# nv-dvl/nerfmatch

Hardware: AMD Instinct MI355X
Metric: rays*samples/sec (higher is better)
Workload: dtype fp16x3 (fp16 MFMA on hi/lo-split fp32 operands, three products per fp32 product, fp32 accumulate; fp32 everywhere else)

## Files before the change

nerfmatch_amd/csrc/nerf_fwd_bf16.hip:

```cpp
#include "nerf_split_chain.h"

namespace {
using namespace nmbf;
using nmsample::HALF_PI_F32, nmsample::SCAN_TILE, nmsample::frustum, nmsample::ray_consts, nmsample::lift_var, nmsample::ipe_fast, nmsample::view_row_value;
using nmsample::alpha_of, nmsample::trans_factor, nmsample::sigmoid, nmsample::scan_before_barrier, nmsample::scan_after_barrier, nmsample::scan_carry;
using nmsample::first_max;
static_assert(TILE == SCAN_TILE, "the compositing scan of nerf_sample.h spans two wavefronts");

template <int PART>
__device__ __forceinline__ void tap_prefetch(Ctx& cx) {
  if constexpr (PART == 0) __builtin_amdgcn_s_barrier();
  const char* src = reinterpret_cast<const char*>(cx.tapw);
#pragma unroll
  for (int q = (PART == 0 ? 0 : 4); q < (PART == 0 ? 4 : 7); ++q) {
    const char* sp = src + q * 4096;
    const float* dp = q < 4 ? cx.tap_ring + q * 1024 : cx.tap_ipe + (q - 4) * 1024;
    const unsigned lds = (unsigned)__builtin_amdgcn_readfirstlane((int)(unsigned)(size_t)(const __attribute__((address_space(3))) float*)dp);
    unsigned m0_saved;
    asm volatile("s_mov_b32 %0, m0\n\ts_mov_b32 m0, %1\n\tglobal_load_lds_dwordx4 %2, off\n\tglobal_load_lds_dwordx4 %2, off offset:1024\n\t"
                 "global_load_lds_dwordx4 %2, off offset:2048\n\tglobal_load_lds_dwordx4 %2, off offset:3072\n\ts_mov_b32 m0, %0"
                 : "=&s"(m0_saved) : "s"(lds), "v"(sp) : "memory");
  }
}

// ... 57 lines not shown
#pragma unroll
    for (int i = 0; i < 8; ++i) s2[8 * b + i] = o[i];
  }
  float s3[16];
#pragma unroll
  for (int b = 0; b < 2; ++b) {
    float o[8], x[8], y[8];
#pragma unroll
    for (int i = 0; i < 8; ++i) { x[i] = s2[8 * b + i]; y[i] = s2[16 + 8 * b + i]; }
    dpp_pairs8(o, x, y, false);
#pragma unroll
    for (int i = 0; i < 8; ++i) s3[8 * b + i] = o[i];
  }
  float lo8[8], hi8[8];
#pragma unroll
  for (int i = 0; i < 8; ++i) { lo8[i] = s3[i]; hi8[i] = s3[8 + i]; }
  quad_add8<2>(lo8); quad_add8<2>(hi8);
  float s4[8];
#pragma unroll
  for (int i = 0; i < 8; ++i) s4[i] = (lane & 2) ? hi8[i] : lo8[i];
  float t8[8] = {s4[0], s4[1], s4[2], s4[3], s4[4], s4[5], s4[6], s4[7]};
  quad_add8<1>(t8);
  return (lane & 1) ? f32x4{t8[4], t8[5], t8[6], t8[7]} : f32x4{t8[0], t8[1], t8[2], t8[3]};
}
__device__ __forceinline__ f32x4 reduce_scatter_32rows(float (&v)[128], int lane) {
  float s1[64];
#pragma unroll
  for (int i = 0; i < 64; ++i) s1[i] = reduce_scatter_step16(v[i], v[64 + i]);
  return reduce_scatter_16pairs(s1, lane);
}

#define NM_MLP_DONE_WAIT() __builtin_amdgcn_s_waitcnt(0x0070)
#define NM_EPI_BARRIER() asm volatile("s_waitcnt lgkmcnt(0)\n\ts_barrier" ::: "memory")
template <int P, bool TAP7 = true>
__device__ __forceinline__ void nerf_fwd_body(const NerfArgs& a) {
  constexpr bool DENS = P == 2 && !TAP7;
  __shared__ __attribute__((aligned(16))) float sm[LDS_TOTAL];
  float* const sm_small = sm + LDS_SMALL;
  float* const ring = sm + LDS_RING;
  float* const sm_ipe = sm + LDS_IPE;
  float* const sm_sigma = sm + LDS_SCR;
  float* const sm_rgb = sm_sigma + TILE;
  float* const sm_t0 = sm_rgb + 3 * TILE;
  float* const sm_t1 = sm_t0 + TILE;
  float* const sm_mean = sm_t1 + TILE;
  float* const sm_dn = sm_mean + 3 * TILE;
  float* const sm_w = sm_dn + TILE;
  float* const sm_misc = sm_w + TILE;
  float* const sm_part = sm_misc + 32;
  float* const sm_feat = sm + LDS_FEAT;
  float* const sm_ex = sm + LDS_EX;
  int* const sm_lray = reinterpret_cast<int*>(sm + LDS_LEFT);
  float* const sm_lT = sm + LDS_LEFT + TILE;
  unsigned* const sm_rng = reinterpret_cast<unsigned*>(sm + LDS_RNG);

  const int tid = threadIdx.x, lane = tid & 63, wave = tid >> 6, s = lane & 31, hi = lane >> 5;
  const bool tail_ok = a.left && !(a.tail_viol && *a.tail_viol != 0);
  const int S = a.S, R = a.R;
  const int Sa = tail_ok ? a.Sa : S;
  const int left = tail_ok ? 1 : 0;
  const int ntiles = tail_ok ? a.ntiles : a.ntiles_full;
  const int SP = Sa < TILE ? Sa : TILE;
  const int nr = TILE / SP;
  const int nchunks = (Sa + TILE - 1) / TILE;
  const bool need_rgb = !(a.flags & NM_NERF_SKIP_RGB);
  const bool feat_max = (a.flags & NM_NERF_FEAT_MAX) != 0;
  const bool need_tap = (a.feat != nullptr) || (a.sfeat != nullptr);
  const int tap = (a.tap < 0 || a.tap > 7) ? 7 : a.tap;
  const int nslots = need_rgb ? NSLOT_FULL : NSLOT_NORGB;
// ... 48 lines not shown
    const float t0 = a.t[(size_t)rc * (S + 1) + sidx];
    const float t1 = a.t[(size_t)rc * (S + 1) + sidx + 1];
    float t_mean, t_var, r_var;
    frustum(t0, t1, radius, t_mean, t_var, r_var);
    float mean[3] = {d0 * t_mean + o0, d1 * t_mean + o1, d2 * t_mean + o2};
    float var[3];
    lift_var(t_var, r_var, dsq, nul, a.var_scale, var);
    if (hi == 0) {
      sm_t0[js] = t0; sm_t1[js] = t1;
      sm_mean[js] = mean[0]; sm_mean[TILE + js] = mean[1]; sm_mean[2 * TILE + js] = mean[2];
      sm_dn[js] = dnorm;
    }

    ring_open<P>(blob_slots, ring, wave, lane);

    {
      const float ipe_scale = sm_small[OFF_INSCALE];
      const float phl = hi ? HALF_PI_F32 : 0.f;
      park_ipe<P>(sm_ipe + wave * (XS * 2 * 64 * 4) + lane * 4, [&](int idx) {
        const int ax = idx % 3;
        const float sc = (float)(1 << (idx / 3));
        float v = ipe_fast(mean[ax] * sc + phl, var[ax], sc);
        if constexpr (P == 2) v *= ipe_scale;
        return v;
      });
    }

    TRACE(2);
    Ctx cx;
    cx.blob_slots = blob_slots; cx.ring = ring; cx.sm_small = sm_small;
    cx.tapw = reinterpret_cast<f32x4*>(a.ws) + ((size_t)blockIdx.x * 4 + wave) * 32 * 64 + lane;
    cx.nslots = nslots; cx.wave = wave; cx.lane = lane; cx.hi = hi; cx.tap = need_tap ? tap : -1; cx.g = 0; cx.sig_part = 0.f;
    cx.vmax = 0.f; cx.rng = sm_rng + tid; cx.sc = 1.f;
    const bool early = TAP7 && need_rgb && !lo_pass && tap == 7 && a.feat && !a.sfeat;
    cx.tap_pref = need_tap && !lo_pass && !early; cx.rgb = need_rgb;
    cx.tap_ring = ring + wave * SLOT_FLOATS; cx.tap_ipe = sm_ipe + wave * (XS * 2 * 64 * 4);
    if constexpr (is_split<P>()) {
      ring_open_wait<P>(cx);
    } else {
      ring_acquire<P>(blob_slots, 0, nslots, ring, wave, lane);
    }
    load_half<P>(cx.opA, ring, lane, 0);
    if constexpr (P == 1) load_half<1>(cx.opB, ring, lane, 1);
    const float* ipe_src = sm_ipe + wave * (XS * 2 * 64 * 4) + lane * 4;

    auto composite_weights = [&]() __attribute__((always_inline)) {
      const int tid2 = launder(threadIdx.x), lane2 = tid2 & 63, wave2 = tid2 >> 6;
      float alpha = 0.f, incl = 1.f;
      if (tid2 < TILE) {
        alpha = alpha_of(sm_sigma[tid2], (sm_t1[tid2] - sm_t0[tid2]) * sm_dn[tid2]);
        incl = scan_before_barrier(trans_factor(alpha), lane2, wave2, SP, sm_misc);
      }
      NM_EPI_BARRIER();
      if (tid2 < TILE) {
        const float excl = scan_after_barrier(incl, lane2, wave2, SP, sm_misc, carryT);
        sm_w[tid2] = alpha * excl;
        const int r2 = tid2 / SP, ray2 = bid * nr + r2;
        if (left && chunk == nchunks - 1 && ray2 < R && tid2 % SP == SP - 1) {
          sm_lray[nleft + r2] = ray2;
          sm_lT[nleft + r2] = excl * trans_factor(alpha);
        }
      }
      if (nchunks > 1) carryT = scan_carry(carryT, sm_misc);
    };
    auto composite_sums = [&]() __attribute__((always_inline)) {
      const int tid2 = launder(threadIdx.x);
      if (tid2 < TILE) {
        const float wgt = sm_w[tid2];
        const int r2 = tid2 / SP, ray2 = bid * nr + r2;
        if (ray2 < R) {
          const int s2 = chunk * TILE + tid2 % SP;
          a.weights[(size_t)ray2 * S + s2] = wgt;
          if (left && chunk == nchunks - 1) {
            for (int k = Sa + 1 + tid2 % SP; k < S; k += SP) a.weights[(size_t)ray2 * S + k] = 0.f;
          }
          if (a.raw && !NM_TRACE) {
            f32x4 rv = {sm_rgb[tid2], sm_rgb[TILE + tid2], sm_rgb[2 * TILE + tid2], sm_sigma[tid2]};
            *reinterpret_cast<f32x4*>(a.raw + ((size_t)ray2 * S + s2) * 4) = rv;
          }
        }
        float pq[8] = {wgt, wgt * sm_rgb[tid2], wgt * sm_rgb[TILE + tid2], wgt * sm_rgb[2 * TILE + tid2],
                       wgt * (0.5f * (sm_t0[tid2] + sm_t1[tid2])), wgt * sm_mean[tid2], wgt * sm_mean[TILE + tid2],
                       wgt * sm_mean[2 * TILE + tid2]};
        nm_half_sum_dpp8(pq);
        if ((tid2 & 31) == 16) {
          *reinterpret_cast<f32x4*>(sm_part + (tid2 >> 5) * 8) = f32x4{pq[0], pq[1], pq[2], pq[3]};
          *reinterpret_cast<f32x4*>(sm_part + (tid2 >> 5) * 8 + 4) = f32x4{pq[4], pq[5], pq[6], pq[7]};
        }
      }
    };
    auto pick_best = [&]() __attribute__((always_inline)) {
      const int tid2 = launder(threadIdx.x);
      if (tid2 < 8 * nr) {
        const int q = tid2 & 7, r2 = tid2 >> 3;
        const float* wv = sm_w + r2 * SP;
        int bi;
        const bool better = first_max(wv, SP, best_w, bi);
        if (q == 0) sm_misc[8 + r2] = better ? __int_as_float(r2 * SP + bi) : __int_as_float(-1);
        if (q >= 5 && better) red_acc = sm_mean[(q - 5) * TILE + r2 * SP + bi];
      }
    };
    auto tap7_early = [&](Ctx& c) __attribute__((always_inline)) {
      const int t2 = launder(threadIdx.x), jl = (t2 >> 6) * 32 + (t2 & 31), hl = (t2 >> 5) & 1;
      const float sigma_raw = (c.sig_part + nm_shfl_xor32(c.sig_part)) + sm_small[OFF_MISC];
      if (hl == 0) sm_sigma[jl] = sigma_raw;
      NM_EPI_BARRIER();
      composite_weights();
      NM_EPI_BARRIER();
      if (feat_max) {
        pick_best();
        NM_EPI_BARRIER();
      }
      const float desc = sm_small[OFF_DESCALE + 7];
      const float wj = sm_w[jl] * desc;
      const int best = feat_max ? __float_as_int(sm_misc[8 + jl / SP]) : -2;
      const float mult = feat_max ? (jl == best ? desc : 0.f) : wj;
      const float* bl = sm_small + OFF_BIAS + 7 * 256 + 4 * hl;
      const float s7 = sm_small[OFF_SCALE + 7];
      float s1[64];
#pragma unroll
      for (int cq = 0; cq < HS; ++cq) {
        const f32x4 b0 = *reinterpret_cast<const f32x4*>(bl + (cq >> 2) * 32 + 8 * (cq & 3));
        const f32x4 b1 = *reinterpret_cast<const f32x4*>(bl + (4 + (cq >> 2)) * 32 + 8 * (cq & 3));
#pragma unroll
        for (int e = 0; e < 4; ++e) {
          const float x = mult * __builtin_fmaxf(__builtin_fmaf(c.hv[4 * cq + e], s7, b0[e]), 0.f);
          const float y = mult * __builtin_fmaxf(__builtin_fmaf(c.hv[64 + 4 * cq + e], s7, b1[e]), 0.f);
          s1[4 * cq + e] = reduce_scatter_step16(x, y);
        }
      }
      const f32x4 sum4 = reduce_scatter_16pairs(s1, jl);
      const int r = jl & 31;
      float* prow = sm_feat + (jl >> 5) * 256 + 4 * hl;
      *reinterpret_cast<f32x4*>(prow + (r >> 2) * 32 + 16 * ((r >> 1) & 1) + 8 * (r & 1)) = sum4;
    };
    const Tap7InRegisters<decltype(tap7_early)> tap7{early, tap7_early};
    f32x16 acc[8];
    ipe_steps<P, true>(acc, cx, ipe_src);
    finish_layer<P>(acc, 0, cx);
    TRACE(3);
#pragma unroll 1
    for (int l = 1; l < 8; ++l) {
      layer_pass<P, DENS>(acc, l, cx, ipe_src, tap7);
      TRACE(3 + l);
    }
    float c_r = 0.f, c_g = 0.f, c_b = 0.f;
    if (!need_rgb) {
      if (cx.tap == 7) dump_tap(7, cx);
      NM_MLP_DONE_WAIT();
      if (cx.tap_pref) tap_prefetch<0>(cx);
      alpha_head(cx);
      if (cx.tap_pref) tap_prefetch<1>(cx);
    } else {
      const int hh = launder(lane) >> 5;
      const float* exr = sm_ex + launder(rl) * 48 + 8 * hh;
      f32x16 av[4];
      if constexpr (DENS) {
        views_hidden<P, true>(av, cx);
        dens_close(cx);
      } else views_hidden<P>(av, cx);
      fold_range<P>(cx, 7);
      bf16x8 exh[VS], exl[VS];
#pragma unroll
      for (int e = 0; e < VS; ++e) {
        float v8[8];
        if (!lo_pass) {
          const f32x4 e0 = *reinterpret_cast<const f32x4*>(exr + 16 * e), e1 = *reinterpret_cast<const f32x4*>(exr + 16 * e + 4);
          v8[0] = e0[0]; v8[1] = e0[1]; v8[2] = e0[2]; v8[3] = e0[3]; v8[4] = e1[0]; v8[5] = e1[1]; v8[6] = e1[2]; v8[7] = e1[3];
        } else {
          const float* rq = a.rays + (size_t)launder(rc) * 12 + 8;
          const float vd0 = rq[0], vd1 = rq[1], vd2 = rq[2];
#pragma unroll
          for (int i = 0; i < 8; ++i) {
            const int f = 16 * e + 8 * hh + i;
            const int ax = f % 3;
            float v = view_row_value(f, ax == 0 ? vd0 : ax == 1 ? vd1 : vd2, a.app_row);
// ... 68 lines not shown
      }
      __syncthreads();
      if (need_tap) {
        const int jl = launder(js), hl = launder(lane) >> 5;
        const f32x4* tw = reinterpret_cast<const f32x4*>(a.ws) + ((size_t)blockIdx.x * 4 + wave2) * 32 * 64 + lane2;
        if (jl < nent) {
          const int ray2 = sm_lray[jl];
          const float desc = sm_small[OFF_DESCALE + tap];
          const float wj = sm_w[jl] * desc;
#pragma unroll 4
          for (int ks = 0; ks < HS; ++ks) {
            const f32x4 ta = tw[(2 * ks) * 64], tb = tw[(2 * ks + 1) * 64];
            const int n0 = (ks >> 1) * 32 + 16 * (ks & 1) + 4 * hl;
            if (a.sfeat) {
              float* dsf = a.sfeat + ((size_t)ray2 * S + Sa) * 256 + n0;
              *reinterpret_cast<f32x4*>(dsf) = ta * desc;
              *reinterpret_cast<f32x4*>(dsf + 8) = tb * desc;
            }
            if (a.feat) {
              float* df = a.feat + (size_t)ray2 * 256 + n0;
#pragma unroll
              for (int e = 0; e < 4; ++e) {
                atomicAdd(df + e, wj * ta[e]);
                atomicAdd(df + 8 + e, wj * tb[e]);
              }
            }
          }
        }
      }
      __syncthreads();
      break;
    }

    if (!early) composite_weights();
    composite_sums();
    NM_EPI_BARRIER();

    if (tid2 < 8 * nr) {
      const int q = tid2 & 7, r2 = tid2 >> 3;
      if (!feat_max || q < 5) {
        float sum = 0.f;
        for (int hw = r2 * (SP / 32); hw < (r2 + 1) * (SP / 32); ++hw) sum += sm_part[hw * 8 + q];
        red_acc += sum;
      }
    }
    if (feat_max && !early) {
      pick_best();
      NM_EPI_BARRIER();
    }

    TRACE(14);
    if (need_tap && !early) {
      const int jl = launder(js), hl = launder(lane) >> 5;
      f32x4 tapv[2 * HS];
      {
        asm volatile("s_waitcnt vmcnt(0)" ::: "memory");
        f32x4 tail[4];
        {
          const f32x4* tw = reinterpret_cast<const f32x4*>(a.ws) + ((size_t)blockIdx.x * 4 + (launder(threadIdx.x) >> 6)) * 32 * 64 + (launder(threadIdx.x) & 63);
#pragma unroll
          for (int i = 0; i < 4; ++i) tail[i] = tw[(28 + i) * 64];
        }
        const float* lr = ring + (launder(threadIdx.x) >> 6) * SLOT_FLOATS + (launder(threadIdx.x) & 63) * 4;
        const float* li = sm_ipe + (launder(threadIdx.x) >> 6) * (XS * 2 * 64 * 4) + (launder(threadIdx.x) & 63) * 4;
#pragma unroll
        for (int c = 0; c < 2 * HS; ++c)
          tapv[c] = c < 16 ? *reinterpret_cast<const f32x4*>(lr + c * 256) : c < 28 ? *reinterpret_cast<const f32x4*>(li + (c - 16) * 256) : tail[c - 28];
      }
      const float desc = sm_small[OFF_DESCALE + tap];
      const float wj = sm_w[jl] * desc;
      const int rsel = jl / SP;
      const int best = feat_max ? __float_as_int(sm_misc[8 + rsel]) : -2;
      float* prow = sm_feat + (jl >> 5) * 256 + 4 * hl;
      if (a.sfeat && ray < R) {
#pragma unroll
        for (int ks = 0; ks < HS; ++ks) {
          const f32x4 ta = tapv[2 * ks], tb = tapv[2 * ks + 1];
          float* dsf = a.sfeat + ((size_t)ray * S + sidx) * 256 + (ks >> 1) * 32 + 16 * (ks & 1) + 4 * hl;
          *reinterpret_cast<f32x4*>(dsf) = ta * desc;
          *reinterpret_cast<f32x4*>(dsf + 8) = tb * desc;
        }
      }
      if (a.feat) {
        float wv[128];
        const float mult = feat_max ? (jl == best ? desc : 0.f) : wj;
#pragma unroll
        for (int c = 0; c < 2 * HS; ++c)
#pragma unroll
          for (int e = 0; e < 4; ++e) wv[4 * c + e] = mult * tapv[c][e];
        const f32x4 sum4 = reduce_scatter_32rows(wv, jl);
        const int r = jl & 31;
        *reinterpret_cast<f32x4*>(prow + (r >> 2) * 32 + 16 * ((r >> 1) & 1) + 8 * (r & 1)) = sum4;
      }
    }
    TRACE(15);
    __syncthreads();
    TRACE(16);
    if (a.feat) {
      const int wpr = SP / 32;
      for (int r2 = 0; r2 < nr; ++r2) {
        float f = 0.f;
        bool any = !feat_max;
        if (feat_max) {
          const int best = __float_as_int(sm_misc[8 + r2]);
          any = best >= 0;
        }
        for (int w2 = 0; w2 < wpr; ++w2) f += sm_feat[(r2 * wpr + w2) * 256 + tid2];
        const int ray2 = bid * nr + r2;
        if (nchunks > 1) {
          if (feat_max) { if (any) feat_run = f; }
          else feat_run += f;
          f = feat_run;
        }
        if (ray2 < R && chunk == nchunks - 1 && (any || nchunks > 1)) a.feat[(size_t)ray2 * 256 + tid2] = f;
      }
    }
    __syncthreads();
  }

  if (lo_pass) {
    nleft = 0;
    continue;
  }
  if (tid < 8 * nr) {
    const int q = tid & 7, r2 = tid >> 3, ray2 = bid * nr + r2;
    const float accv = __shfl(red_acc, lane & ~7, 64);
    if (ray2 < R) {
      if (q == 0) { if (a.acc) a.acc[ray2] = red_acc; }
      else if (q <= 3) { if (a.rgb && need_rgb) a.rgb[(size_t)ray2 * 3 + (q - 1)] = a.white_bg ? red_acc + (1.0f - accv) : red_acc; }
      else if (q == 4) { if (a.depth) a.depth[ray2] = red_acc; }
      else { if (a.pts) a.pts[(size_t)ray2 * 3 + (q - 5)] = red_acc; }
    }
  }
  TRACE(17);
  if (left) nleft += (R - bid * nr) < nr ? (R - bid * nr) : nr;
  bid += gridDim.x;
  }
  if constexpr (P == 2) {
    __syncthreads();
    if (a.status && tid < NRANGE) {
      unsigned m = 0u;
      for (int i = 0; i < 256; ++i) m = max(m, sm_rng[tid * 256 + ((i + 32 * tid) & 255)]);
      if (m) atomicMax(reinterpret_cast<unsigned*>(a.status) + 1 + tid, m);
      if (m >= __float_as_uint(F16_MAX)) atomicOr(a.status, 1);
    }
  }
}

__global__ void __launch_bounds__(256, 1) nerf_fwd_bf16x3_kernel(NerfArgs a) { nerf_fwd_body<0>(a); }
__global__ void __launch_bounds__(256, 1) nerf_fwd_fp16x1_kernel(NerfArgs a) { nerf_fwd_body<1>(a); }
__global__ void __launch_bounds__(256, 1) nerf_fwd_fp16x3_kernel(NerfArgs a) { nerf_fwd_body<2, false>(a); }
__global__ void __launch_bounds__(256, 1) nerf_fwd_fp16x3_tap7_kernel(NerfArgs a) { nerf_fwd_body<2, true>(a); }

}

extern "C" size_t nm_nerf_workspace_bytes_bf16x3(void) { return (size_t)WS_WORKGROUPS * TILE * 256 * sizeof(float); }

static int nerf_fwd_split(int mode, const void* blob, const float* rays, const float* t, const float* app_row, int R, int S, int tap_layer,
                          int white_bg, float var_scale, int flags, float* weights, float* feat, float* pts, float* rgb, float* depth,
                          float* acc, float* raw, float* sample_feat, void* workspace, const int* zero_tail_violation, nmStream_t stream,
                          int* status = nullptr) {
  NM_CHECK_ARG(blob && rays && t && weights && R > 0 && S > 0);
  if (!(S == 32 || S == 64 || (S % 128) == 0)) return NM_ERR_UNSUPPORTED;
  if (tap_layer > 7) return NM_ERR_ARG;
  if ((feat || sample_feat) && !workspace) return NM_ERR_WORKSPACE;
  NerfArgs a;
  a.ws = (float*)workspace;
  a.blob = (const char*)blob; a.rays = rays; a.t = t; a.app_row = app_row;
  a.weights = weights; a.feat = feat; a.pts = pts; a.rgb = rgb; a.depth = depth; a.acc = acc; a.raw = raw; a.sfeat = sample_feat;
  a.R = R; a.S = S; a.tap = tap_layer; a.white_bg = white_bg; a.flags = flags; a.var_scale = var_scale;
  a.status = status;
  const bool zero_tail = (flags & NM_NERF_ZERO_TAIL) && (S == 64 || S == 128 || (S >= 256 && S % 256 == 0)) && !raw && !sample_feat &&
                         !(flags & NM_NERF_FEAT_MAX);
  a.Sa = zero_tail ? S / 2 : S;
  a.left = zero_tail ? 1 : 0;
  const int SP = a.Sa < TILE ? a.Sa : TILE, nr = TILE / SP;
  a.ntiles = (R + nr - 1) / nr;
  const int SPf = S < TILE ? S : TILE, nrf = TILE / SPf;
  a.ntiles_full = (R + nrf - 1) / nrf;
  a.tail_viol = zero_tail ? zero_tail_violation : nullptr;
  const int ncu = nm_stream_cus(stream);
  const int grid = a.ntiles < ncu ? a.ntiles : (ncu < WS_WORKGROUPS ? ncu : WS_WORKGROUPS);
  if (mode == 1) nerf_fwd_fp16x1_kernel<<<grid, 256, 0, (hipStream_t)stream>>>(a);
  else if (mode == 2) {
    const bool tap7_early = !(flags & NM_NERF_SKIP_RGB) && (tap_layer < 0 || tap_layer == 7) && feat && !sample_feat;
    if (tap7_early) nerf_fwd_fp16x3_tap7_kernel<<<grid, 256, 0, (hipStream_t)stream>>>(a);
    else nerf_fwd_fp16x3_kernel<<<grid, 256, 0, (hipStream_t)stream>>>(a);
  }
  else nerf_fwd_bf16x3_kernel<<<grid, 256, 0, (hipStream_t)stream>>>(a);
  return nm_launch_status();
}

extern "C" int nm_nerf_fwd_bf16x3(const void* blob, const float* rays, const float* t, const float* app_row, int R, int S,
                                  int tap_layer, int white_bg, float var_scale, int flags, float* weights, float* feat, float* pts,
                                  float* rgb, float* depth, float* acc, float* raw, float* sample_feat, void* workspace,
                                  const int* zero_tail_violation, nmStream_t stream) {
  return nerf_fwd_split(0, blob, rays, t, app_row, R, S, tap_layer, white_bg, var_scale, flags, weights, feat, pts, rgb, depth, acc, raw,
                        sample_feat, workspace, zero_tail_violation, stream);
}

extern "C" int nm_nerf_fwd_fp16x1(const void* blob, const float* rays, const float* t, const float* app_row, int R, int S,
                                  int tap_layer, int white_bg, float var_scale, int flags, float* weights, float* feat, float* pts,
                                  float* rgb, float* depth, float* acc, float* raw, float* sample_feat, void* workspace,
                                  const int* zero_tail_violation, nmStream_t stream) {
  return nerf_fwd_split(1, blob, rays, t, app_row, R, S, tap_layer, white_bg, var_scale, flags, weights, feat, pts, rgb, depth, acc, raw,
                        sample_feat, workspace, zero_tail_violation, stream);
}

extern "C" int nm_nerf_fwd_fp16x3(const void* blob, const float* rays, const float* t, const float* app_row, int R, int S,
                                  int tap_layer, int white_bg, float var_scale, int flags, float* weights, float* feat, float* pts,
                                  float* rgb, float* depth, float* acc, float* raw, float* sample_feat, void* workspace,
                                  const int* zero_tail_violation, int* status, nmStream_t stream) {
  return nerf_fwd_split(2, blob, rays, t, app_row, R, S, tap_layer, white_bg, var_scale, flags, weights, feat, pts, rgb, depth, acc, raw,
                        sample_feat, workspace, zero_tail_violation, stream, status);
}
```

nerfmatch_amd/csrc/nerf_points_bf16.hip:

```cpp
#include "nerf_split_chain.h"

namespace {
using namespace nmbf;
using nmsample::HALF_PI_F32, nmsample::frustum, nmsample::ray_consts, nmsample::lift_var, nmsample::ipe_exact, nmsample::view_row_value;

struct PointsArgs {
  const char* blob;
  const float* xi;
  const float* xd;
  const float* g4;
  float* out4;
  float* g_xi0;
  float* g_xi5;
  float* g_xd;
  u32x4* gates;
  int n, ntiles;
  const float* rays;
  const float* z;
  const float* app_row;
  int S, Sa;
  float* feats;
  const float* tap_w;
  const float* tap_g;
  int tap;
// ... 26 lines not shown
#pragma unroll 1
  for (int bid = blockIdx.x; bid < a.ntiles; bid += gridDim.x) {
    __syncthreads();
    const int sample = bid * TILE + wave * 32 + s;
    const size_t sc = (size_t)(sample < a.n ? sample : a.n - 1);
    ring_open<P>(blob_slots, ring, wave, lane);
    float vdir[3] = {0.f, 0.f, 0.f};
    {
      float* dst = sm_ipe + wave * (XS * 2 * 64 * 4) + lane * 4;
      if constexpr (RAYS) {
        const int r = (int)(sc / (size_t)a.Sa), si = (int)(sc % (size_t)a.Sa);
        const float* rp = a.rays + (size_t)r * 12;
        const float t0 = a.z[(size_t)r * (a.S + 1) + si], t1 = a.z[(size_t)r * (a.S + 1) + si + 1];
        vdir[0] = rp[8]; vdir[1] = rp[9]; vdir[2] = rp[10];
        float t_mean, t_var, r_var, dsq[3], nul[3], dnorm, mean[3], var[3];
        frustum(t0, t1, rp[11], t_mean, t_var, r_var);
        ray_consts(rp + 3, dsq, nul, dnorm);
        lift_var(t_var, r_var, dsq, nul, 0.f, var);
#pragma unroll
        for (int ax = 0; ax < 3; ++ax) mean[ax] = rp[ax] + t_mean * vdir[ax];
        const float phl = hi ? HALF_PI_F32 : 0.f;
        park_ipe<P>(dst, [&](int idx) {
          const float scl = (float)(1 << (idx / 3));
          return ipe_exact(mean[idx % 3] * scl + phl, var[idx % 3], scl);
        });
      } else {
        const float* row = a.xi + sc * 96 + 45 * hi;
        park_ipe<P>(dst, [&](int idx) { return row[idx]; });
      }
    }
    Ctx cx;
    cx.blob_slots = blob_slots; cx.ring = ring; cx.sm_small = sm_small; cx.tapw = nullptr;
    cx.nslots = NSLOT_FULL; cx.wave = wave; cx.lane = lane; cx.hi = hi; cx.tap = -1; cx.g = 0; cx.sig_part = 0.f;
    cx.vmax = 0.f; cx.rng = nullptr; cx.sc = 1.f; cx.tap_pref = false; cx.rgb = true; cx.tap_ring = nullptr; cx.tap_ipe = nullptr;
    cx.gptr = a.gates + (size_t)bid * 9 * 256 + tid;
    cx.gbits[0] = cx.gbits[1] = cx.gbits[2] = cx.gbits[3] = 0u;
    ring_open_wait<P>(cx);
    load_half<P>(cx.opA, ring, lane, 0);
    const float* ipe_src = sm_ipe + wave * (XS * 2 * 64 * 4) + lane * 4;
    f32x16 acc[8];
    ipe_steps<P, true>(acc, cx, ipe_src);
    finish_layer<P>(acc, 0, cx);
    const bool tapped = a.feats != nullptr;
#pragma unroll 1
    for (int l = 1; l < 8; ++l) {
      if (tapped && l - 1 == a.tap) dump_tap_rows(l - 1, cx, a.feats + sc * 256, launder(lane) >> 5, sample < a.n);
      layer_pass<P>(acc, l, cx, ipe_src);
    }
    if (tapped && a.tap == 7) dump_tap_rows(7, cx, a.feats + sc * 256, launder(lane) >> 5, sample < a.n);
    f32x16 av[4];
    views_hidden<P>(av, cx);
    cx.gptr[7 * 256] = u32x4{cx.gbits[0], cx.gbits[1], cx.gbits[2], cx.gbits[3]};
    const int hh = launder(lane) >> 5;
    {
      const float* row = a.xd + sc * 48 + 8 * hh;
      bf16x8 exh[VS], exl[VS];
#pragma unroll
      for (int e = 0; e < VS; ++e) {
        float v8[8];
        if constexpr (RAYS) {
#pragma unroll
          for (int i = 0; i < 8; ++i) {
            const int f = 16 * e + 8 * hh + i;
            const int ax = f % 3;
            v8[i] = view_row_value(f, ax == 0 ? vdir[0] : ax == 1 ? vdir[1] : vdir[2], a.app_row);
          }
        } else {
// ... 124 lines not shown
#pragma unroll
    for (int r = 0; r < 16; ++r) cx.hv[ob * 16 + r] = acc_read(acc[ob][r]);
}
__device__ __forceinline__ void store_acc4(const f32x16 (&av)[4], float* dst_row, int ncol, int hh, bool valid) {
#pragma unroll
  for (int ob = 0; ob < 4; ++ob)
#pragma unroll
    for (int q = 0; q < 4; ++q) {
      const int c = 32 * ob + 8 * q + 4 * hh;
      const f32x4 v = {acc_read(av[ob][4 * q + 0]), acc_read(av[ob][4 * q + 1]), acc_read(av[ob][4 * q + 2]), acc_read(av[ob][4 * q + 3])};
      if (valid && c + 3 < ncol) *reinterpret_cast<f32x4*>(dst_row + c) = v;
    }
}

__device__ __forceinline__ void points_bwd_body(const PointsArgs& a) {
  __shared__ __attribute__((aligned(16))) float sm[LDS_IPE];
  float* const sm_small = sm + LDS_SMALL;
  float* const ring = sm + LDS_RING;
  const int tid = threadIdx.x, lane = tid & 63, wave = tid >> 6, s = lane & 31, hi = lane >> 5;
  const char* const blob_slots = a.blob + (size_t)SMALL_PAD * 4;
  for (int i = tid; i < SMALL / 4; i += 256) reinterpret_cast<f32x4*>(sm_small)[i] = reinterpret_cast<const f32x4*>(a.blob)[i];
#pragma unroll 1
  for (int bid = blockIdx.x; bid < a.ntiles; bid += gridDim.x) {
    __syncthreads();
    const int sample = bid * TILE + wave * 32 + s;
    const bool valid = sample < a.n;
    const size_t sc = (size_t)(valid ? sample : a.n - 1);
    ring_open<0>(blob_slots, ring, wave, lane);
    const u32x4* gt = a.gates + (size_t)bid * 9 * 256 + tid;
    const f32x4 g4 = *reinterpret_cast<const f32x4*>(a.g4 + sc * 4);
    Ctx cx;
    cx.blob_slots = blob_slots; cx.ring = ring; cx.sm_small = sm_small; cx.tapw = nullptr;
    cx.nslots = NSLOT_BWD; cx.wave = wave; cx.lane = lane; cx.hi = hi; cx.tap = -1; cx.g = launder_s(0); cx.sig_part = 0.f;
    cx.vmax = 0.f; cx.rng = nullptr; cx.sc = 1.f; cx.tap_pref = false; cx.rgb = true; cx.tap_ring = nullptr; cx.tap_ipe = nullptr; cx.gptr = nullptr;
    const int hh = launder(lane) >> 5;
    {
      const u32x4 gv = gt[8 * 256];
      const float* wr = sm_small + OFF_WRGB + 4 * hh;
#pragma unroll
      for (int ob = 0; ob < 4; ++ob)
#pragma unroll
        for (int q = 0; q < 4; ++q) {
          const f32x4 wr4 = *reinterpret_cast<const f32x4*>(wr + ob * 32 + 8 * q);
          const f32x4 wg4 = *reinterpret_cast<const f32x4*>(wr + 128 + ob * 32 + 8 * q);
          const f32x4 wb4 = *reinterpret_cast<const f32x4*>(wr + 256 + ob * 32 + 8 * q);
#pragma unroll
          for (int e = 0; e < 4; ++e) {
            const float g = NM_FMA(wb4[e], g4[2], NM_FMA(wg4[e], g4[1], wr4[e] * g4[0]));
            const int bit = 16 * (ob & 1) + 4 * q + e;
            cx.hv[ob * 16 + 4 * q + e] = __int_as_float(__float_as_int(g) & __builtin_amdgcn_sbfe((int)gv[ob >> 1], bit, 1));
          }
        }
    }
    ring_open_wait<0>(cx);
    load_half<0>(cx.opA, ring, lane, 0);
    const u32x4 none = {0u, 0u, 0u, 0u};
    f32x16 acc[8];
    {
      f32x16 av[4];
      make_unit0_b<false>(cx, none);
      bwd_product<4, 8, false>(av, cx, none);
      store_acc4(av, a.g_xd + sc * 48, 48, hh, valid);
    }
    make_unit0_b<false>(cx, none);
    bwd_product<8, 8, false>(acc, cx, none);
    take_acc8(acc, cx);
    {
// ... 93 lines not shown
```

nerfmatch_amd/csrc/nerf_split_chain.h:

```cpp
#pragma once
#include "nerf_bf16_common.h"

namespace nmbf {

template <int P> constexpr bool is_bf16() { return P == 0 || P == 4; }
template <int P> constexpr bool has_gates() { return P == 4; }
typedef _Float16 f16x8 __attribute__((ext_vector_type(8)));
typedef _Float16 f16x2 __attribute__((ext_vector_type(2)));
template <int P>
__device__ __forceinline__ f32x16 mfma_p(const bf16x8& a, const bf16x8& b, const f32x16& c) {
  if constexpr (is_bf16<P>()) return MFMA_BF16(a, b, c);
  else return __builtin_amdgcn_mfma_f32_32x32x16_f16(__builtin_bit_cast(f16x8, a), __builtin_bit_cast(f16x8, b), c, 0, 0, 0);
}
template <int P> constexpr bool is_split() { return P != 1; }
template <int P> constexpr int slot_bytes() { return is_split<P>() ? SLOT_BYTES : SLOT_BYTES / 2; }
template <int P> constexpr int slot_floats() { return slot_bytes<P>() / 4; }
template <int P> constexpr int ring_slots() { return is_split<P>() ? NRING : 2 * NRING; }
template <int P> constexpr int ring_ahead() { return is_split<P>() ? 4 : 6; }
constexpr float F16_MAX = 65504.0f;
__device__ __forceinline__ void split8_f16(const float (&v)[8], bf16x8& hi, bf16x8& lo) {
  f16x8 h8, l8;
#pragma unroll
  for (int i = 0; i < 8; ++i) {
    const float c = __builtin_amdgcn_fmed3f(v[i], -F16_MAX, F16_MAX);
// ... 78 lines not shown

__device__ __forceinline__ void ring_acquire_pair(const char* blob_slots, int g, float* ring, int wave, int lane) {
  NM_WAIT_VMCNT(6);
  __builtin_amdgcn_s_barrier();
  dma_slot<1>(blob_slots, g + 6, ring, wave, lane);
  dma_slot<1>(blob_slots, g + 7, ring, wave, lane);
}

struct OpHalf {
  bf16x8 h[4], l[4];
};

template <int P>
__device__ __forceinline__ void load_half(OpHalf& d, const float* slot, int lane, int p) {
  const u32x4* s4 = reinterpret_cast<const u32x4*>(slot) + lane;
#pragma unroll
  for (int o = 0; o < 4; ++o) {
    if constexpr (is_split<P>()) {
      d.h[o] = __builtin_bit_cast(bf16x8, s4[((4 * p + o) * 2 + 0) * 64]);
      d.l[o] = __builtin_bit_cast(bf16x8, s4[((4 * p + o) * 2 + 1) * 64]);
    } else {
      d.h[o] = __builtin_bit_cast(bf16x8, s4[(4 * p + o) * 64]);
    }
  }
}

struct Ctx {
  const char* blob_slots;
  float* ring;
  const float* sm_small;
  f32x4* tapw;
  bool tap_pref;
  bool rgb;
  float* tap_ring;
  float* tap_ipe;
  int nslots, wave, lane, hi;
  int tap;
  int g;
  unsigned dma_voff;
  unsigned dma_lds;
  OpHalf opA;
  OpHalf opB;
  f32x4 hb0, hb1;
  Unit xn;
  float sig_part;
  float dp[4];
  float dv[3], dw[3];
  f32x4 nb0, nb1;
  float sc;
  float vmax;
  unsigned* rng;
  u32x4* gptr;
  unsigned gbits[4];
  float hv[128];
};

template <int P>
__device__ __forceinline__ void ring_request(const Ctx& cx, int g, int j) {
  const int slot = g + 2 + (j >> 2);
  const char* base = cx.blob_slots + (size_t)slot * slot_bytes<P>();
  const unsigned lds = cx.dma_lds + (unsigned)(slot & (ring_slots<P>() - 1)) * slot_bytes<P>();
  unsigned m0_saved;
#define NM_DMA_PIECE(OFS)                                                                                                        \
  asm volatile("s_mov_b32 %0, m0\n\ts_mov_b32 m0, %1\n\tglobal_load_lds_dwordx4 %2, %3 offset:" #OFS "\n\ts_mov_b32 m0, %0" \
               : "=&s"(m0_saved) : "s"(lds), "v"(cx.dma_voff), "s"(base) : "memory")
  switch (j & 3) {
// ... 322 lines not shown
      p3 = NM_FMA(__builtin_fmaxf(__builtin_fmaf(cx.hv[ob * 16 + 4 * q + 3], s7, b[3]), 0.f), w4v[3], p3);
    }
  cx.sig_part = (p0 + p1) + (p2 + p3);
}

__device__ __forceinline__ void dens_open(Ctx& cx) {
  const float* bl = cx.sm_small + OFF_BIAS + 7 * 256 + 4 * cx.hi;
  const float* wa = cx.sm_small + OFF_WALPHA + 4 * cx.hi;
  const f32x4 b0 = *reinterpret_cast<const f32x4*>(bl), b1 = *reinterpret_cast<const f32x4*>(bl + 8);
  const f32x4 w0 = *reinterpret_cast<const f32x4*>(wa), w1 = *reinterpret_cast<const f32x4*>(wa + 8);
  float v[8];
#pragma unroll
  for (int j = 0; j < 4; ++j) {
    v[j] = __builtin_fmaxf(__builtin_fmaf(cx.hv[j], cx.sc, b0[j]), 0.f);
    v[4 + j] = __builtin_fmaxf(__builtin_fmaf(cx.hv[4 + j], cx.sc, b1[j]), 0.f);
  }
#pragma unroll
  for (int j = 0; j < 4; ++j) cx.dp[j] = NM_FMA(v[j], w0[j], 0.f);
  cx.dp[0] = NM_FMA(v[4], w1[0], cx.dp[0]);
#pragma unroll
  for (int j = 0; j < 3; ++j) { cx.dv[j] = v[5 + j]; cx.dw[j] = w1[1 + j]; }
}
struct DensTail {
  Ctx& cx;
  __device__ __forceinline__ void seq(int c) {
    if (c == 1) {
#pragma unroll
      for (int j = 0; j < 3; ++j) UnitWork<2, true>::dens_fma(cx.dp[1 + j], cx.dv[j], cx.dw[j]);
    }
  }
};
__device__ __forceinline__ void dens_close(Ctx& cx) { cx.sig_part = (cx.dp[0] + cx.dp[1]) + (cx.dp[2] + cx.dp[3]); }

__device__ __forceinline__ void dump_tap(int lo, Ctx& cx) {
  const float* bl = cx.sm_small + OFF_BIAS + lo * 256 + 4 * cx.hi;
  const float sl = cx.sm_small[OFF_SCALE + lo];
  auto* tp = (__attribute__((address_space(1))) f32x4*)cx.tapw;
#pragma unroll
  for (int ob = 0; ob < 8; ++ob) {
    f32x4 v[4];
#pragma unroll
    for (int q = 0; q < 4; ++q) {
      const f32x4 b = *reinterpret_cast<const f32x4*>(bl + ob * 32 + 8 * q);
#pragma unroll
      for (int e = 0; e < 4; ++e) v[q][e] = __builtin_fmaxf(__builtin_fmaf(cx.hv[ob * 16 + 4 * q + e], sl, b[e]), 0.f);
    }
#pragma unroll
    for (int q = 0; q < 4; ++q) tp[q * 64] = v[q];
    tp += 256;
    pin(tp);
  }
}

__device__ __forceinline__ bf16x8 load_op1(const float* slot, int lane, int blk) {
  return __builtin_bit_cast(bf16x8, (reinterpret_cast<const u32x4*>(slot) + lane)[blk * 64]);
}
#define NM_SB __builtin_amdgcn_sched_barrier(0)
template <bool FIRST, bool ACQ, class Work>
__device__ __forceinline__ void slot_step8_one(f32x16 (&acc)[8], Ctx& cx, const bf16x8& x, Work work) {
  const f32x16 zero = {0.f, 0.f, 0.f, 0.f, 0.f, 0.f, 0.f, 0.f, 0.f, 0.f, 0.f, 0.f, 0.f, 0.f, 0.f, 0.f};
  const int g = cx.g;
  const OpHalf A = cx.opA, B = cx.opB;
  const float* nxt = ring_slot<1>(cx.ring, g + 1);
  acc[0] = mfma_p<1>(A.h[0], x, FIRST ? zero : acc[0]); NM_SB;
  if constexpr (ACQ) ring_acquire_pair(cx.blob_slots, g, cx.ring, cx.wave, cx.lane);
  NM_SB;
  acc[1] = mfma_p<1>(A.h[1], x, FIRST ? zero : acc[1]); NM_SB;
  cx.opA.h[0] = load_op1(nxt, cx.lane, 0); cx.opA.h[1] = load_op1(nxt, cx.lane, 1); work.prefetch(); NM_SB;
  acc[2] = mfma_p<1>(A.h[2], x, FIRST ? zero : acc[2]); NM_SB;
  cx.opA.h[2] = load_op1(nxt, cx.lane, 2); cx.opA.h[3] = load_op1(nxt, cx.lane, 3); NM_SB;
  acc[3] = mfma_p<1>(A.h[3], x, FIRST ? zero : acc[3]); NM_SB;
  cx.opB.h[0] = load_op1(nxt, cx.lane, 4); cx.opB.h[1] = load_op1(nxt, cx.lane, 5); NM_SB;
  acc[4] = mfma_p<1>(B.h[0], x, FIRST ? zero : acc[4]); NM_SB;
  cx.opB.h[2] = load_op1(nxt, cx.lane, 6); cx.opB.h[3] = load_op1(nxt, cx.lane, 7); NM_SB;
  acc[5] = mfma_p<1>(B.h[1], x, FIRST ? zero : acc[5]); NM_SB;
  work(0); work(1); NM_SB;
  acc[6] = mfma_p<1>(B.h[2], x, FIRST ? zero : acc[6]); NM_SB;
  work(2); work(3); work(4); NM_SB;
// ... 187 lines not shown
}

template <int P, bool FIRST>
__device__ __forceinline__ void ipe_steps(f32x16 (&acc)[8], Ctx& cx, const float* ipe_src, int l = FIRST ? 0 : 5) {
  auto operand = [&](int m, bf16x8& ph, bf16x8& pl) {
    ph = __builtin_bit_cast(bf16x8, *reinterpret_cast<const u32x4*>(ipe_src + (is_split<P>() ? (m * 2 + 0) : m) * 256));
    pl = ph;
    if constexpr (is_split<P>()) pl = __builtin_bit_cast(bf16x8, *reinterpret_cast<const u32x4*>(ipe_src + (m * 2 + 1) * 256));
  };
  if constexpr (P == 2) {
    bf16x8 ph, pl, qh, ql;
    operand(0, ph, pl);
#pragma unroll
    for (int m = 0; m < XS; m += 2) {
      if (m == 0) slot_step8<P, FIRST, true>(acc, cx, ph, pl, IpeFetch<17>{ipe_src, m + 1, qh, ql});
      else slot_step8<P, false, true, true>(acc, cx, ph, pl, IpeFetch<6>{ipe_src, m + 1, qh, ql});
      if (m + 2 == XS) slot_step8<P, false, false>(acc, cx, qh, ql, AccTake<P>{acc, cx, l});
      else slot_step8<P, false, false, true>(acc, cx, qh, ql, IpeFetch<4>{ipe_src, m + 2, ph, pl});
    }
    return;
  }
#pragma unroll
  for (int m = 0; m < XS; m += 2) {
    bf16x8 ph, pl;
    operand(m, ph, pl);
    if (m == 0) slot_step8<P, FIRST, true>(acc, cx, ph, pl, NoWork{});
    else slot_step8<P, false, true>(acc, cx, ph, pl, NoWork{});
    operand(m + 1, ph, pl);
    if (m + 2 == XS) slot_step8<P, false, false>(acc, cx, ph, pl, AccTake<P>{acc, cx, l});
    else slot_step8<P, false, false>(acc, cx, ph, pl, NoWork{});
  }
}

struct Tap7Workspace {
  static constexpr bool on = false;
  __device__ __forceinline__ void fn(Ctx&) const {}
};
template <class F>
struct Tap7InRegisters {
  bool on;
  F fn;
};

template <int P, bool DENS = false, class Tap7 = Tap7Workspace>
__device__ __forceinline__ void layer_pass(f32x16 (&acc)[8], int l, Ctx& cx, const float* ipe_src, const Tap7& tap7 = Tap7()) {
  if (l - 1 == cx.tap) dump_tap(l - 1, cx);
#pragma unroll
  for (int ks = 0; ks < HS; ks += 2) {
    {
      const Unit xc = cx.xn;
      if (ks == 0) slot_step8<P, true, true>(acc, cx, __builtin_bit_cast(bf16x8, xc.h), __builtin_bit_cast(bf16x8, xc.l), unit_work<P>(ks + 1, l - 1, cx, cx.xn));
      else slot_step8<P, false, true, request_early<P>()>(acc, cx, __builtin_bit_cast(bf16x8, xc.h), __builtin_bit_cast(bf16x8, xc.l), unit_work<P>(ks + 1, l - 1, cx, cx.xn));
    }
    {
      const Unit xc = cx.xn;
      if (ks + 2 < HS) slot_step8<P, false, false, request_early<P>()>(acc, cx, __builtin_bit_cast(bf16x8, xc.h), __builtin_bit_cast(bf16x8, xc.l), unit_work<P>(ks + 2, l - 1, cx, cx.xn));
      else slot_step8<P, false, false>(acc, cx, __builtin_bit_cast(bf16x8, xc.h), __builtin_bit_cast(bf16x8, xc.l), AccTake<P>{acc, cx, l});
    }
  }
  fold_range<P>(cx, l - 1);
  if constexpr (has_gates<P>()) {
    cx.gptr[(l - 1) * 256] = u32x4{cx.gbits[0], cx.gbits[1], cx.gbits[2], cx.gbits[3]};
    cx.gbits[0] = cx.gbits[1] = cx.gbits[2] = cx.gbits[3] = 0u;
  }
  if (l == 5) ipe_steps<P, false>(acc, cx, ipe_src);
  finish_layer<P>(acc, l, cx);
  if (l == 7) {
    if (cx.rgb) {
      if (cx.tap == 7 && !tap7.on) dump_tap(7, cx);
      if constexpr (DENS) dens_open(cx);
      else alpha_head(cx);
      if (tap7.on) tap7.fn(cx);
    }
  }
}

}
```

Measured before the change: 397.3 million.

## Keep layer-7 tap activations in registers through compositing instead of early tap kernel

Removes the separate fp16x3 tap7 kernel variant and its in-layer early compositing lambda. When the tap is layer 7 with feature output, the pre-activation hidden values now stay in cx.hv. The bias, scale and ReLU are applied after the normal compositing pass, so the workspace dump and reload are skipped. This drops the duplicated composite barriers in the MLP epilogue and a separate kernel instantiation. The cost is that cx.hv must stay live across the compositing code, which raises register pressure.

```diff
diff --git a/nerfmatch_amd/csrc/nerf_fwd_bf16.hip b/nerfmatch_amd/csrc/nerf_fwd_bf16.hip
--- a/nerfmatch_amd/csrc/nerf_fwd_bf16.hip
+++ b/nerfmatch_amd/csrc/nerf_fwd_bf16.hip
@@ -113,9 +113,9 @@
 
 #define NM_MLP_DONE_WAIT() __builtin_amdgcn_s_waitcnt(0x0070)
 #define NM_EPI_BARRIER() asm volatile("s_waitcnt lgkmcnt(0)\n\ts_barrier" ::: "memory")
-template <int P, bool TAP7 = true>
+template <int P>
 __device__ __forceinline__ void nerf_fwd_body(const NerfArgs& a) {
-  constexpr bool DENS = P == 2 && !TAP7;
+  constexpr bool DENS = P == 2;
   __shared__ __attribute__((aligned(16))) float sm[LDS_TOTAL];
   float* const sm_small = sm + LDS_SMALL;
   float* const ring = sm + LDS_RING;
@@ -230,8 +230,9 @@
     cx.tapw = reinterpret_cast<f32x4*>(a.ws) + ((size_t)blockIdx.x * 4 + wave) * 32 * 64 + lane;
     cx.nslots = nslots; cx.wave = wave; cx.lane = lane; cx.hi = hi; cx.tap = need_tap ? tap : -1; cx.g = 0; cx.sig_part = 0.f;
     cx.vmax = 0.f; cx.rng = sm_rng + tid; cx.sc = 1.f;
-    const bool early = TAP7 && need_rgb && !lo_pass && tap == 7 && a.feat && !a.sfeat;
-    cx.tap_pref = need_tap && !lo_pass && !early; cx.rgb = need_rgb;
+    const bool tap_regs = need_rgb && !lo_pass && tap == 7 && a.feat && !a.sfeat;
+    cx.tap_regs = tap_regs;
+    cx.tap_pref = need_tap && !lo_pass && !tap_regs; cx.rgb = need_rgb;
     cx.tap_ring = ring + wave * SLOT_FLOATS; cx.tap_ipe = sm_ipe + wave * (XS * 2 * 64 * 4);
     if constexpr (is_split<P>()) {
       ring_open_wait<P>(cx);
@@ -298,48 +299,13 @@
         if (q >= 5 && better) red_acc = sm_mean[(q - 5) * TILE + r2 * SP + bi];
       }
     };
-    auto tap7_early = [&](Ctx& c) __attribute__((always_inline)) {
-      const int t2 = launder(threadIdx.x), jl = (t2 >> 6) * 32 + (t2 & 31), hl = (t2 >> 5) & 1;
-      const float sigma_raw = (c.sig_part + nm_shfl_xor32(c.sig_part)) + sm_small[OFF_MISC];
-      if (hl == 0) sm_sigma[jl] = sigma_raw;
-      NM_EPI_BARRIER();
-      composite_weights();
-      NM_EPI_BARRIER();
-      if (feat_max) {
-        pick_best();
-        NM_EPI_BARRIER();
-      }
-      const float desc = sm_small[OFF_DESCALE + 7];
-      const float wj = sm_w[jl] * desc;
-      const int best = feat_max ? __float_as_int(sm_misc[8 + jl / SP]) : -2;
-      const float mult = feat_max ? (jl == best ? desc : 0.f) : wj;
-      const float* bl = sm_small + OFF_BIAS + 7 * 256 + 4 * hl;
-      const float s7 = sm_small[OFF_SCALE + 7];
-      float s1[64];
-#pragma unroll
-      for (int cq = 0; cq < HS; ++cq) {
-        const f32x4 b0 = *reinterpret_cast<const f32x4*>(bl + (cq >> 2) * 32 + 8 * (cq & 3));
-        const f32x4 b1 = *reinterpret_cast<const f32x4*>(bl + (4 + (cq >> 2)) * 32 + 8 * (cq & 3));
-#pragma unroll
-        for (int e = 0; e < 4; ++e) {
-          const float x = mult * __builtin_fmaxf(__builtin_fmaf(c.hv[4 * cq + e], s7, b0[e]), 0.f);
-          const float y = mult * __builtin_fmaxf(__builtin_fmaf(c.hv[64 + 4 * cq + e], s7, b1[e]), 0.f);
-          s1[4 * cq + e] = reduce_scatter_step16(x, y);
-        }
-      }
-      const f32x4 sum4 = reduce_scatter_16pairs(s1, jl);
-      const int r = jl & 31;
-      float* prow = sm_feat + (jl >> 5) * 256 + 4 * hl;
-      *reinterpret_cast<f32x4*>(prow + (r >> 2) * 32 + 16 * ((r >> 1) & 1) + 8 * (r & 1)) = sum4;
-    };
-    const Tap7InRegisters<decltype(tap7_early)> tap7{early, tap7_early};
     f32x16 acc[8];
     ipe_steps<P, true>(acc, cx, ipe_src);
     finish_layer<P>(acc, 0, cx);
     TRACE(3);
 #pragma unroll 1
     for (int l = 1; l < 8; ++l) {
-      layer_pass<P, DENS>(acc, l, cx, ipe_src, tap7);
+      layer_pass<P, DENS>(acc, l, cx, ipe_src);
       TRACE(3 + l);
     }
     float c_r = 0.f, c_g = 0.f, c_b = 0.f;
@@ -474,7 +440,7 @@
       break;
     }
 
-    if (!early) composite_weights();
+    composite_weights();
     composite_sums();
     NM_EPI_BARRIER();
 
@@ -486,16 +452,25 @@
         red_acc += sum;
       }
     }
-    if (feat_max && !early) {
+    if (feat_max) {
       pick_best();
       NM_EPI_BARRIER();
     }
 
     TRACE(14);
-    if (need_tap && !early) {
+    if (need_tap) {
       const int jl = launder(js), hl = launder(lane) >> 5;
-      f32x4 tapv[2 * HS];
-      {
+      if (tap_regs) {
+        const float* bl = sm_small + OFF_BIAS + 7 * 256 + 4 * hl;
+        const float s7 = sm_small[OFF_SCALE + 7];
+        f32x4 b7[2 * HS];
+#pragma unroll
+        for (int c = 0; c < 2 * HS; ++c) b7[c] = *reinterpret_cast<const f32x4*>(bl + (c >> 2) * 32 + 8 * (c & 3));
+#pragma unroll
+        for (int c = 0; c < 2 * HS; ++c)
+#pragma unroll
+          for (int e = 0; e < 4; ++e) cx.hv[4 * c + e] = tap_act(cx.hv[4 * c + e], s7, b7[c][e]);
+      } else {
         asm volatile("s_waitcnt vmcnt(0)" ::: "memory");
         f32x4 tail[4];
         {
@@ -506,8 +481,11 @@
         const float* lr = ring + (launder(threadIdx.x) >> 6) * SLOT_FLOATS + (launder(threadIdx.x) & 63) * 4;
         const float* li = sm_ipe + (launder(threadIdx.x) >> 6) * (XS * 2 * 64 * 4) + (launder(threadIdx.x) & 63) * 4;
 #pragma unroll
-        for (int c = 0; c < 2 * HS; ++c)
-          tapv[c] = c < 16 ? *reinterpret_cast<const f32x4*>(lr + c * 256) : c < 28 ? *reinterpret_cast<const f32x4*>(li + (c - 16) * 256) : tail[c - 28];
+        for (int c = 0; c < 2 * HS; ++c) {
+          const f32x4 row = c < 16 ? *reinterpret_cast<const f32x4*>(lr + c * 256) : c < 28 ? *reinterpret_cast<const f32x4*>(li + (c - 16) * 256) : tail[c - 28];
+#pragma unroll
+          for (int e = 0; e < 4; ++e) cx.hv[4 * c + e] = row[e];
+        }
       }
       const float desc = sm_small[OFF_DESCALE + tap];
       const float wj = sm_w[jl] * desc;
@@ -517,7 +495,8 @@
       if (a.sfeat && ray < R) {
 #pragma unroll
         for (int ks = 0; ks < HS; ++ks) {
-          const f32x4 ta = tapv[2 * ks], tb = tapv[2 * ks + 1];
+          const f32x4 ta = {cx.hv[8 * ks], cx.hv[8 * ks + 1], cx.hv[8 * ks + 2], cx.hv[8 * ks + 3]};
+          const f32x4 tb = {cx.hv[8 * ks + 4], cx.hv[8 * ks + 5], cx.hv[8 * ks + 6], cx.hv[8 * ks + 7]};
           float* dsf = a.sfeat + ((size_t)ray * S + sidx) * 256 + (ks >> 1) * 32 + 16 * (ks & 1) + 4 * hl;
           *reinterpret_cast<f32x4*>(dsf) = ta * desc;
           *reinterpret_cast<f32x4*>(dsf + 8) = tb * desc;
@@ -529,7 +508,7 @@
 #pragma unroll
         for (int c = 0; c < 2 * HS; ++c)
 #pragma unroll
-          for (int e = 0; e < 4; ++e) wv[4 * c + e] = mult * tapv[c][e];
+          for (int e = 0; e < 4; ++e) wv[4 * c + e] = mult * cx.hv[4 * c + e];
         const f32x4 sum4 = reduce_scatter_32rows(wv, jl);
         const int r = jl & 31;
         *reinterpret_cast<f32x4*>(prow + (r >> 2) * 32 + 16 * ((r >> 1) & 1) + 8 * (r & 1)) = sum4;
@@ -591,8 +570,7 @@
 
 __global__ void __launch_bounds__(256, 1) nerf_fwd_bf16x3_kernel(NerfArgs a) { nerf_fwd_body<0>(a); }
 __global__ void __launch_bounds__(256, 1) nerf_fwd_fp16x1_kernel(NerfArgs a) { nerf_fwd_body<1>(a); }
-__global__ void __launch_bounds__(256, 1) nerf_fwd_fp16x3_kernel(NerfArgs a) { nerf_fwd_body<2, false>(a); }
-__global__ void __launch_bounds__(256, 1) nerf_fwd_fp16x3_tap7_kernel(NerfArgs a) { nerf_fwd_body<2, true>(a); }
+__global__ void __launch_bounds__(256, 1) nerf_fwd_fp16x3_kernel(NerfArgs a) { nerf_fwd_body<2>(a); }
 
 }
 
@@ -624,11 +602,7 @@
   const int ncu = nm_stream_cus(stream);
   const int grid = a.ntiles < ncu ? a.ntiles : (ncu < WS_WORKGROUPS ? ncu : WS_WORKGROUPS);
   if (mode == 1) nerf_fwd_fp16x1_kernel<<<grid, 256, 0, (hipStream_t)stream>>>(a);
-  else if (mode == 2) {
-    const bool tap7_early = !(flags & NM_NERF_SKIP_RGB) && (tap_layer < 0 || tap_layer == 7) && feat && !sample_feat;
-    if (tap7_early) nerf_fwd_fp16x3_tap7_kernel<<<grid, 256, 0, (hipStream_t)stream>>>(a);
-    else nerf_fwd_fp16x3_kernel<<<grid, 256, 0, (hipStream_t)stream>>>(a);
-  }
+  else if (mode == 2) nerf_fwd_fp16x3_kernel<<<grid, 256, 0, (hipStream_t)stream>>>(a);
   else nerf_fwd_bf16x3_kernel<<<grid, 256, 0, (hipStream_t)stream>>>(a);
   return nm_launch_status();
 }
diff --git a/nerfmatch_amd/csrc/nerf_points_bf16.hip b/nerfmatch_amd/csrc/nerf_points_bf16.hip
--- a/nerfmatch_amd/csrc/nerf_points_bf16.hip
+++ b/nerfmatch_amd/csrc/nerf_points_bf16.hip
@@ -82,7 +82,7 @@
     Ctx cx;
     cx.blob_slots = blob_slots; cx.ring = ring; cx.sm_small = sm_small; cx.tapw = nullptr;
     cx.nslots = NSLOT_FULL; cx.wave = wave; cx.lane = lane; cx.hi = hi; cx.tap = -1; cx.g = 0; cx.sig_part = 0.f;
-    cx.vmax = 0.f; cx.rng = nullptr; cx.sc = 1.f; cx.tap_pref = false; cx.rgb = true; cx.tap_ring = nullptr; cx.tap_ipe = nullptr;
+    cx.vmax = 0.f; cx.rng = nullptr; cx.sc = 1.f; cx.tap_pref = false; cx.tap_regs = false; cx.rgb = true; cx.tap_ring = nullptr; cx.tap_ipe = nullptr;
     cx.gptr = a.gates + (size_t)bid * 9 * 256 + tid;
     cx.gbits[0] = cx.gbits[1] = cx.gbits[2] = cx.gbits[3] = 0u;
     ring_open_wait<P>(cx);
@@ -273,7 +273,7 @@
     Ctx cx;
     cx.blob_slots = blob_slots; cx.ring = ring; cx.sm_small = sm_small; cx.tapw = nullptr;
     cx.nslots = NSLOT_BWD; cx.wave = wave; cx.lane = lane; cx.hi = hi; cx.tap = -1; cx.g = launder_s(0); cx.sig_part = 0.f;
-    cx.vmax = 0.f; cx.rng = nullptr; cx.sc = 1.f; cx.tap_pref = false; cx.rgb = true; cx.tap_ring = nullptr; cx.tap_ipe = nullptr; cx.gptr = nullptr;
+    cx.vmax = 0.f; cx.rng = nullptr; cx.sc = 1.f; cx.tap_pref = false; cx.tap_regs = false; cx.rgb = true; cx.tap_ring = nullptr; cx.tap_ipe = nullptr; cx.gptr = nullptr;
     const int hh = launder(lane) >> 5;
     {
       const u32x4 gv = gt[8 * 256];
diff --git a/nerfmatch_amd/csrc/nerf_split_chain.h b/nerfmatch_amd/csrc/nerf_split_chain.h
--- a/nerfmatch_amd/csrc/nerf_split_chain.h
+++ b/nerfmatch_amd/csrc/nerf_split_chain.h
@@ -134,6 +134,7 @@
   f32x4* tapw;
   bool tap_pref;
   bool rgb;
+  bool tap_regs;
   float* tap_ring;
   float* tap_ipe;
   int nslots, wave, lane, hi;
@@ -522,6 +523,7 @@
 };
 __device__ __forceinline__ void dens_close(Ctx& cx) { cx.sig_part = (cx.dp[0] + cx.dp[1]) + (cx.dp[2] + cx.dp[3]); }
 
+__device__ __forceinline__ float tap_act(float v, float s_tap, float b) { return __builtin_fmaxf(__builtin_fmaf(v, s_tap, b), 0.f); }
 __device__ __forceinline__ void dump_tap(int lo, Ctx& cx) {
   const float* bl = cx.sm_small + OFF_BIAS + lo * 256 + 4 * cx.hi;
   const float sl = cx.sm_small[OFF_SCALE + lo];
@@ -533,7 +535,7 @@
     for (int q = 0; q < 4; ++q) {
       const f32x4 b = *reinterpret_cast<const f32x4*>(bl + ob * 32 + 8 * q);
 #pragma unroll
-      for (int e = 0; e < 4; ++e) v[q][e] = __builtin_fmaxf(__builtin_fmaf(cx.hv[ob * 16 + 4 * q + e], sl, b[e]), 0.f);
+      for (int e = 0; e < 4; ++e) v[q][e] = tap_act(cx.hv[ob * 16 + 4 * q + e], sl, b[e]);
     }
 #pragma unroll
     for (int q = 0; q < 4; ++q) tp[q * 64] = v[q];
@@ -787,18 +789,8 @@
   }
 }
 
-struct Tap7Workspace {
-  static constexpr bool on = false;
-  __device__ __forceinline__ void fn(Ctx&) const {}
-};
-template <class F>
-struct Tap7InRegisters {
-  bool on;
-  F fn;
-};
-
-template <int P, bool DENS = false, class Tap7 = Tap7Workspace>
-__device__ __forceinline__ void layer_pass(f32x16 (&acc)[8], int l, Ctx& cx, const float* ipe_src, const Tap7& tap7 = Tap7()) {
+template <int P, bool DENS = false>
+__device__ __forceinline__ void layer_pass(f32x16 (&acc)[8], int l, Ctx& cx, const float* ipe_src) {
   if (l - 1 == cx.tap) dump_tap(l - 1, cx);
 #pragma unroll
   for (int ks = 0; ks < HS; ks += 2) {
@@ -822,12 +814,11 @@
   finish_layer<P>(acc, l, cx);
   if (l == 7) {
     if (cx.rgb) {
-      if (cx.tap == 7 && !tap7.on) dump_tap(7, cx);
+      if (cx.tap == 7 && !cx.tap_regs) dump_tap(7, cx);
       if constexpr (DENS) dens_open(cx);
       else alpha_head(cx);
-      if (tap7.on) tap7.fn(cx);
-    }
-  }
-}
-
-}
+    }
+  }
+}
+
+}
```

New measurement: 396.2 million. No clear change (-0.3%).
